# ctxnn/GenConViT

Measured on AMD Instinct MI355X. Metric: frames/sec (224x224, ed+vae forward), higher is better.
Workload: dtype f16

## Files before the change

genconvit_amd/_lib.py:

```python
from __future__ import annotations

import ctypes
import ctypes.util
import json
import os
import threading

_HERE = os.path.dirname(os.path.abspath(__file__))
LIB_PATH = os.environ.get("GCV_LIB_PATH") or os.path.join(_HERE, "lib", "libgenconvit_hip.so")

GCV_F32, GCV_BF16, GCV_F16 = 0, 1, 2
ACT_NONE, ACT_RELU, ACT_GELU, ACT_LEAKY = 0, 1, 2, 3
A_PLAIN, A_IM2COL3_POOL, A_IM2COL3_S2 = 0, 1, 2
EPI_BIAS_ACT, EPI_RESID, EPI_POOL4, EPI_CONVT, EPI_SPLITK = 0, 1, 2, 3, 4

c_void_p, c_int, c_int64, c_float, c_char_p, c_size_t = (ctypes.c_void_p, ctypes.c_int, ctypes.c_int64,
                                                         ctypes.c_float, ctypes.c_char_p, ctypes.c_size_t)


class TensorDesc(ctypes.Structure):
    _fields_ = [("name", c_char_p), ("data", c_void_p), ("numel", c_int64), ("on_device", c_int)]


class GemmArgs(ctypes.Structure):
# ... 46 lines not shown
    "gcv_frame_hist": (c_int, [c_void_p, c_int, c_int, c_int, c_int, c_void_p, c_void_p]),
    "gcv_hist_diff": (c_int, [c_void_p, c_int, c_int, c_void_p, c_void_p]),
    "gcv_frame_cells": (c_int, [c_void_p, c_int, c_int, c_int, c_int, c_void_p, c_void_p]),
    "gcv_blend_fit": (c_int, [c_void_p, c_int, c_int, c_int, c_void_p, c_void_p]),
    "gcv_hist_diff_lag": (c_int, [c_void_p, c_int, c_int, c_int, c_void_p, c_void_p]),
    "gcv_face_quality": (c_int, [c_void_p, c_int, c_int, c_int, c_void_p, c_int, c_int, c_void_p, c_void_p]),
    "gcv_face_signature": (c_int, [c_void_p, c_int, c_int, c_int, c_void_p, c_int, c_void_p, c_void_p]),
    "gcv_sig_link": (c_int, [c_void_p, c_void_p, c_int, c_int, c_void_p, c_void_p]),
    "gcv_vote_segments": (c_int, [c_void_p, c_int, c_int, c_void_p, c_int, c_void_p, c_void_p]),
    "gcv_vote_windows": (c_int, [c_void_p, c_int, c_int, c_void_p, c_int, c_void_p, c_void_p, c_void_p]),
    "gcv_tap_set": (c_int, [c_void_p, c_char_p, c_void_p, c_size_t]),
    "gcv_tap_clear": (c_int, [c_void_p]),
    "gcv_tap_written": (c_int, [c_void_p, c_char_p]),
    "gcv_profile_enable": (c_int, [c_void_p, c_int]),
    "gcv_profile_report": (c_char_p, [c_void_p]),
    "gcv_k_gemm": (c_int, [c_int, c_int, c_int, ctypes.POINTER(GemmArgs), c_void_p]),
    "gcv_gemm_plan": (c_int, [c_int, c_int, c_int, ctypes.POINTER(GemmArgs), c_void_p]),
    "gcv_k_stem_ln": (c_int, [c_int, c_void_p, c_int64, c_int64, c_int64, c_int64, c_void_p, c_void_p, c_void_p,
                              c_void_p, c_void_p, c_int, c_int, c_int, c_float, c_void_p]),
    "gcv_k_stem_ln_c": (c_int, [c_int, c_void_p, c_int64, c_int64, c_int64, c_int64, c_void_p, c_void_p, c_void_p,
                                c_void_p, c_void_p, c_int, c_int, c_int, c_int, c_float, c_void_p]),
    "gcv_k_dwconv7_ln": (c_int, [c_int, c_void_p, c_void_p, c_void_p, c_void_p, c_void_p, c_void_p, c_int, c_int,
                                 c_int, c_int, c_float, c_void_p]),
    "gcv_dw_plan": (c_int, [c_int, c_int, c_int, c_int, c_int, c_int, c_void_p]),
    "gcv_convnext_res_ok": (c_int, [c_int, c_int]),
    "gcv_k_ln_patchify": (c_int, [c_int, c_void_p, c_void_p, c_void_p, c_void_p, c_int, c_int, c_int, c_int, c_float,
                                  c_void_p]),
    "gcv_k_layernorm_rows": (c_int, [c_int, c_void_p, c_void_p, c_void_p, c_void_p, c_int64, c_int, c_float, c_void_p]),
    "gcv_k_pool_ln": (c_int, [c_int, c_void_p, c_void_p, c_void_p, c_void_p, c_int, c_int, c_int, c_float, c_void_p]),
    "gcv_k_pool_ln_rows": (c_int, [c_int, c_void_p, c_void_p, c_void_p, c_void_p, c_int, c_int, c_int, c_float, c_int, c_int,
                                   c_int, c_void_p]),
    "gcv_k_conv3_first": (c_int, [c_int, c_void_p, c_int64, c_int64, c_int64, c_int64, c_void_p, c_void_p, c_void_p,
                                  c_int, c_int, c_int, c_int, c_int, c_void_p]),
    "gcv_k_convt2_small": (c_int, [c_int, c_void_p, c_void_p, c_void_p, c_void_p, c_int, c_int, c_int, c_int, c_void_p]),
    "gcv_k_reparam": (c_int, [c_int, c_void_p, c_int, c_void_p, c_void_p, c_void_p, c_void_p, c_int, c_int, c_void_p]),
    "gcv_k_head_tail": (c_int, [c_int, c_void_p, c_void_p, c_void_p, c_void_p, c_int, c_int, c_void_p]),
    "gcv_k_head_tail_splitk": (c_int, [c_int, c_void_p, c_int, c_void_p, c_int, c_void_p, c_void_p, c_void_p, c_int, c_int,
                                       c_void_p]),
    "gcv_k_resize_mse": (c_int, [c_int, c_void_p, c_void_p, c_void_p, c_void_p, c_void_p, c_int, c_void_p]),
    "gcv_k_swin_window_attn": (c_int, [c_int, c_void_p, c_void_p, c_void_p, c_int, c_int, c_int, c_int, c_int, c_int,
                                       c_void_p]),
    "gcv_k_patch_merge_ln": (c_int, [c_int, c_void_p, c_void_p, c_void_p, c_void_p, c_int, c_int, c_int, c_int, c_float,
                                     c_void_p]),
    "gcv_k_mean_tokens": (c_int, [c_int, c_void_p, c_void_p, c_int, c_int, c_int, c_void_p]),
    "gcv_k_head_bwd": (c_int, [c_int, c_void_p, c_int, c_void_p, c_void_p, c_void_p, c_void_p, c_void_p, c_void_p, c_void_p,
                               c_int, c_int, c_void_p]),
# ... 879 lines not shown
```

genconvit_amd/csrc/api.hip:

```cpp
#include "../../include/genconvit_hip.h"

#include <dlfcn.h>

#include <cstdio>
#include <cstdlib>
#include <cstring>
#include <map>
#include <mutex>
#include <set>
#include <sstream>
#include <vector>

#include "cam.h"
#include "cam_bwd.h"
#include "cnx_mlp.h"
#include "gemm.h"
#include "kernels.h"
#include "net.h"

namespace gcv {
static thread_local std::string g_err;
void set_error(const std::string& msg) { g_err = msg; }
const char* get_error() { return g_err.c_str(); }

// ... 592 lines not shown
  };
  DISPATCH_DT(dtype, put(gemm_plan<T>(p, g, a_mode, epi)));
}

int gcv_k_stem_ln(int dtype, const void* x, int64_t sb, int64_t sc, int64_t sy, int64_t sx, const float* wp,
                  const float* bias, const float* lnw, const float* lnb, void* out, int nimg, int Ho, int Wo,
                  float eps, gcv_stream s) {
  DISPATCH_DT(dtype, launch_stem_ln<T>((const T*)x, sb, sc, sy, sx, wp, bias, lnw, lnb, (T*)out, nimg, Ho, Wo, eps,
                                       (hipStream_t)s));
}

int gcv_k_stem_ln_c(int dtype, const void* x, int64_t sb, int64_t sc, int64_t sy, int64_t sx, const float* wp,
                    const float* bias, const float* lnw, const float* lnb, void* out, int nimg, int Ho, int Wo, int C,
                    float eps, gcv_stream s) {
  DISPATCH_DT(dtype, launch_stem_ln<T>((const T*)x, sb, sc, sy, sx, wp, bias, lnw, lnb, (T*)out, nimg, Ho, Wo, eps,
                                       (hipStream_t)s, C));
}

int gcv_k_dwconv7_ln(int dtype, const void* x, const float* wdw, const float* bdw, const float* lnw,
                     const float* lnb, void* y, int nimg, int H, int W, int C, float eps, gcv_stream s) {
  DISPATCH_DT(dtype, launch_dwconv7_ln<T>((const T*)x, wdw, bdw, lnw, lnb, (T*)y, nimg, H, W, C, eps, (hipStream_t)s));
}

int gcv_dw_plan(int dtype, int nimg, int H, int W, int C, int aligned, int* out5) {
  GCV_REQUIRE(out5, "null out5");
  DwPlan p;
  auto put = [&](int rc) {
    if (rc == 0) { out5[0] = (int)p.kind; out5[1] = p.grid; out5[2] = p.block; out5[3] = p.lds; out5[4] = p.band_rows; }
    return rc;
  };
  DISPATCH_DT(dtype, put(dw_plan<T>(p, nimg, H, W, C, aligned != 0)));
}

int gcv_convnext_res_ok(int arch, int res) { return cnx_res_ok(arch, res) ? 1 : 0; }

int gcv_k_ln_patchify(int dtype, const void* x, const float* w, const float* b, void* out, int nimg, int H, int W,
                      int C, float eps, gcv_stream s) {
  DISPATCH_DT(dtype, launch_ln_patchify<T>((const T*)x, w, b, (T*)out, nimg, H, W, C, eps, (hipStream_t)s));
}

int gcv_k_layernorm_rows(int dtype, const void* x, const float* w, const float* b, void* out, int64_t rows, int C,
                         float eps, gcv_stream s) {
  DISPATCH_DT(dtype, launch_layernorm_rows<T>((const T*)x, w, b, (T*)out, rows, C, eps, (hipStream_t)s));
}

int gcv_k_pool_ln(int dtype, const void* x, const float* w, const float* b, void* out, int nimg, int HW, int C,
// ... 240 lines not shown
```

genconvit_amd/csrc/dwconv_impl.h:

```cpp
#pragma once
#include <algorithm>
#include <type_traits>

#include "dwconv_mfma.h"
#include "dwconv_pair.h"
#include "dwconv_roll.h"
#include "kernels.h"

namespace gcv {

constexpr int64_t kDwMfmaMinImageRows = 14 * 256;

template <DwKind K, int C_ = 0, int N_ = 0> struct DwShape {
  static constexpr DwKind kind = K;
  static constexpr int C = C_, N = N_;
};

template <typename T, class F> int dw_select(int nimg, int H, int W, int C, bool aligned, F&& f) {
  GCV_REQUIRE(nimg > 0 && H > 0 && W > 0, "dwconv: empty");
  const int ns = W % 7 == 0 ? W / 7 : 0;
  auto go = [&](auto sh) -> int {
    typedef decltype(sh) S;
    DwPlan p;
    p.kind = S::kind; p.C = C;
    if constexpr (S::kind == DwKind::Tile) {
      const int tiles = C == 96 ? 2 : 1;
      p.block = tiles * C;
      p.lds = tiles * 49 * (C + 2) * 4;
      p.grid = cdiv(nimg * cdiv(H, 7) * cdiv(W, 7), tiles);
    } else if constexpr (S::kind == DwKind::Tiny || S::kind == DwKind::TinyPair) {
// ... 53 lines not shown
  return -3;
}

template <typename T> int dw_plan(DwPlan& p, int nimg, int H, int W, int C, bool aligned) {
  return dw_select<T>(nimg, H, W, C, aligned, [&](const DwPlan& q, auto) { p = q; return 0; });
}

template <typename T>
int launch_dwconv7_ln(const T* x, const float* wdw, const float* bdw, const float* lnw, const float* lnb, T* y,
                      int nimg, int H, int W, int C, float eps, hipStream_t s) {
  const bool aligned = ((reinterpret_cast<uintptr_t>(x) | reinterpret_cast<uintptr_t>(y)) & 15u) == 0;
  return dw_select<T>(nimg, H, W, C, aligned, [&](const DwPlan& p, auto sh) -> int {
    typedef decltype(sh) S;
    auto band = [&](auto k) {
      return dw_launch(p, k, s, x, wdw, bdw, lnw, lnb, y, H, p.band_rows, cdiv(H, p.band_rows), eps);
    };
    if constexpr (S::kind == DwKind::Roll) return band(dwconv7_ln_roll_kernel<T, S::C, S::N>);
    else if constexpr (S::kind == DwKind::Mfma) return band(dwconv7_ln_mfma_kernel<T, S::C, S::N>);
    else if constexpr (S::kind == DwKind::Pair) return band(dwconv7_ln_pair_kernel<T, S::C, S::N>);
    else return launch_dw_tile<T>(p, x, wdw, bdw, lnw, lnb, y, nimg, H, W, eps, s);
  });
}

#define GCV_INSTANTIATE_DW(T)                                                                                        \
  template int dw_plan<T>(DwPlan&, int, int, int, int, bool);                                                        \
  template int launch_dwconv7_ln<T>(const T*, const float*, const float*, const float*, const float*, T*, int, int,   \
                                    int, int, float, hipStream_t);

}
```

genconvit_amd/csrc/dwconv_mfma.h:

```cpp
#pragma once
#include "dwconv_roll.h"

namespace gcv {


template <typename T, int C, int NS> struct DwMfmaLds {
  static constexpr int W = 7 * NS;
  static constexpr int NXG = (W + 15) / 16;
  static constexpr int RP = 16 * NXG + 8;
  static constexpr int PITCH = 2 * C + 8;
  static constexpr int SLOT = RP * PITCH;
  static constexpr int IN_BYTES = 3 * SLOT;
  static constexpr int SP = C + 4;
  static constexpr int SVAL_BYTES = 2 * W * SP * 4;
  static constexpr int bytes = IN_BYTES + SVAL_BYTES;
  static constexpr int NTASK = (C / 16) * NXG;
  static constexpr int NMW = 12;
  static constexpr int TPW = NTASK / NMW;
  static constexpr int NCONV = NMW * 64;
  static constexpr int NLN = 256;
  static constexpr int NT = NCONV + NLN;
  static_assert(NTASK % NMW == 0 && TPW >= 1 && NXG % TPW == 0, "a wave's tasks are x groups of one channel group");
  static_assert(PITCH % 8 == 0 && PITCH % 32 == 8, "pitch");
};

typedef float dwm_f32x4 __attribute__((ext_vector_type(4)));
template <typename T> struct Mfma4;
template <> struct Mfma4<half_t> {
  typedef _Float16 v4 __attribute__((ext_vector_type(4)));
  static __device__ __forceinline__ dwm_f32x4 run(uint2 a, uint2 b, dwm_f32x4 c) {
    return __builtin_amdgcn_mfma_f32_4x4x4f16(__builtin_bit_cast(v4, a), __builtin_bit_cast(v4, b), c, 0, 0, 0);
  }
};
template <> struct Mfma4<bf16_t> {
  typedef short v4 __attribute__((ext_vector_type(4)));
  static __device__ __forceinline__ dwm_f32x4 run(uint2 a, uint2 b, dwm_f32x4 c) {
    return __builtin_amdgcn_mfma_f32_4x4x4bf16_1k(__builtin_bit_cast(v4, a), __builtin_bit_cast(v4, b), c, 0, 0, 0);
  }
};

template <typename T, int C, int NS>
__global__ void __launch_bounds__((DwMfmaLds<T, C, NS>::NT), 4)
dwconv7_ln_mfma_kernel(const T* __restrict__ x, const float* __restrict__ wdw ,
                       const float* __restrict__ bdw, const float* __restrict__ lnw, const float* __restrict__ lnb,
                       T* __restrict__ y, int H, int band_rows, int nbands, float eps) {
  static_assert(sizeof(T) == 2, "16-bit storage (fp32 storage: dwconv_roll.h)");
  typedef DwElem<T> EL;
  typedef DwMfmaLds<T, C, NS> LY;
  constexpr int NCONV = LY::NCONV, NLN = LY::NLN;
  constexpr int W = LY::W, P = W, NXG = LY::NXG, TPW = LY::TPW, PITCH = LY::PITCH, SLOT = LY::SLOT, SP = LY::SP;
  constexpr int EPC = EL::EPC;
  extern __shared__ __attribute__((aligned(16))) unsigned char dwm_lds[];
  unsigned char* const in_ring = dwm_lds;
  float* const sval_ring = reinterpret_cast<float*>(dwm_lds + LY::IN_BYTES);

  const int tid = threadIdx.x;
  const int wg = xcd_remap(blockIdx.x, gridDim.x);
  const int band = wg % nbands, img = wg / nbands;
  const int ob = band * band_rows;
  const int nrows = min(band_rows, H - ob);
  const int r0 = ob - 3;
  const int nit = nrows + 6;
  const int it0 = max(0, -r0);
  constexpr int row_bytes = W * C * (int)sizeof(T);
  const int64_t img_elems = (int64_t)H * W * C;
  auto row_ok = [&](int it) { const int r = r0 + it; return it < nit && r >= 0 && r < H; };

  for (int i = tid; i < LY::IN_BYTES / 16; i += LY::NT) reinterpret_cast<u32x4*>(in_ring)[i] = u32x4{0u, 0u, 0u, 0u};
  __syncthreads();

  if (tid < NCONV) {
    const int lane = tid & 63;
    const int wave = __builtin_amdgcn_readfirstlane(tid >> 6);
    const int t0 = wave * TPW;
    const int cg = t0 / NXG, xg0 = t0 % NXG;
    const int cb = lane >> 2, n = lane & 3;
    const int c = 16 * cg + cb;
    uint2 ta[7][3];
#pragma unroll
    for (int ky = 0; ky < 7; ++ky)
// ... 195 lines not shown
      __builtin_amdgcn_sched_barrier(0);
    };

    if (row_ok(it0)) { stage_load(it0); stage_write(0); }
    if (row_ok(it0 + 1)) { stage_load(it0 + 1); stage_write(1); }
    if (row_ok(it0 + 2)) stage_load(it0 + 2);
    GCV_LDS_BARRIER();
    int wslot = 2;
    for (int it = it0; it < nit; ++it) {
      if (row_ok(it + 2)) stage_write(wslot);
      wslot = (wslot == 2) ? 0 : wslot + 1;
      if (row_ok(it + 3)) stage_load(it + 3);
      DW_STAMP(lid == 0 && it == GCV_DW_STAMP_IT, 8); DW_STAMP(lid == 0 && it == GCV_DW_STAMP_IT, 9); DW_STAMP(lid == 0 && it == GCV_DW_STAMP_IT, 10);
      DW_STAMP(lid == NLN - 64 && it == GCV_DW_STAMP_IT, 26);
      if (it >= 7) ln_row(ob + it - 7, (it - 1) & 1);
      DW_STAMP(lid == 0 && it == GCV_DW_STAMP_IT, 13); DW_STAMP(lid == NLN - 64 && it == GCV_DW_STAMP_IT, 27);
      GCV_LDS_BARRIER();
      DW_STAMP(lid == 0 && it == GCV_DW_STAMP_IT, 14); DW_STAMP(lid == NLN - 64 && it == GCV_DW_STAMP_IT, 28);
    }
    ln_row(ob + nit - 7, (nit - 1) & 1);
  }
}

}
```

genconvit_amd/csrc/dwconv_roll.h:

```cpp
#pragma once
#include <type_traits>

#include "common.h"

namespace gcv {

template <typename T> struct DwElem;
template <> struct DwElem<float> {
  static constexpr int EPC = 4;
  __device__ static __forceinline__ u32x4 pack(const float (&v)[4]) {
    return u32x4{__builtin_bit_cast(uint32_t, v[0]), __builtin_bit_cast(uint32_t, v[1]),
                 __builtin_bit_cast(uint32_t, v[2]), __builtin_bit_cast(uint32_t, v[3])};
  }
};
template <> struct DwElem<half_t> {
  static constexpr int EPC = 8;
  __device__ static __forceinline__ float lo(uint32_t v) { return (float)__builtin_bit_cast(_Float16, (uint16_t)v); }
  __device__ static __forceinline__ float hi(uint32_t v) { return (float)__builtin_bit_cast(_Float16, (uint16_t)(v >> 16)); }
};
template <> struct DwElem<bf16_t> {
  static constexpr int EPC = 8;
  __device__ static __forceinline__ float lo(uint32_t v) { return __builtin_bit_cast(float, v << 16); }
  __device__ static __forceinline__ float hi(uint32_t v) { return __builtin_bit_cast(float, v & 0xffff0000u); }
};
// ... 24 lines not shown
  asm volatile("ds_read_b32 %0, %1 offset:%2" : "=v"(dst) : "v"(addr), "n"(OFF));
}
template <int C, int S, int S1> __device__ __forceinline__ void dw_read_row(float (&nxt)[13], uint32_t addr) {
  if constexpr (S < S1) {
    static_assert(S * C * 4 < 65536, "ds offset field");
    dw_lds_rd<S * C * 4>(nxt[S], addr);
    dw_read_row<C, S + 1, S1>(nxt, addr);
  }
}

template <typename T, int C, int NS> struct DwRollLds {
  static constexpr int P = 7 * NS;
  static constexpr int HP = (NS == 1) ? 0 : 3;
  static constexpr int IN_ROW = (P + 2 * HP) * C;
  static constexpr int IN_BYTES = 3 * IN_ROW * 4;
  static constexpr int SVAL_BYTES = 2 * P * C * 4;
  static constexpr int bytes = IN_BYTES + SVAL_BYTES;
  static constexpr int NCONV = NS * C;
  static constexpr int NLN = NCONV / 3;
  static constexpr int NT = NCONV + NLN;
};

template <typename T, int C, int NS>
__global__ void __launch_bounds__((DwRollLds<T, C, NS>::NT), 4)
dwconv7_ln_roll_kernel(const T* __restrict__ x, const float* __restrict__ wdw ,
                       const float* __restrict__ bdw, const float* __restrict__ lnw, const float* __restrict__ lnb,
                       T* __restrict__ y, int H, int band_rows, int nbands, float eps) {
  typedef DwElem<T> EL;
  typedef DwRollLds<T, C, NS> LY;
  constexpr bool FULLW = (NS == 1);
  constexpr int NCONV = LY::NCONV, NLN = LY::NLN;
  constexpr int W = 7 * NS;
  constexpr int P = LY::P, HP = LY::HP, IN_ROW = LY::IN_ROW;
  constexpr int EPC = EL::EPC;
  constexpr int S0 = FULLW ? 3 : 0, S1 = FULLW ? 10 : 13;
  extern __shared__ __attribute__((aligned(16))) unsigned char dwr_lds[];
  float* const in_ring = reinterpret_cast<float*>(dwr_lds);
  float* const sval_ring = reinterpret_cast<float*>(dwr_lds + LY::IN_BYTES);

  const int tid = threadIdx.x;
  const int wg = xcd_remap(blockIdx.x, gridDim.x);
  const int band = wg % nbands, img = wg / nbands;
  const int ob = band * band_rows;
  const int nrows = min(band_rows, H - ob);
  const int r0 = ob - 3;
  const int nit = nrows + 6;
  const int it0 = max(0, -r0);
  constexpr int row_bytes = W * C * (int)sizeof(T);
  const int64_t img_elems = (int64_t)H * W * C;

  auto row_ok = [&](int it) { const int r = r0 + it; return it < nit && r >= 0 && r < H; };

  if (tid < NCONV) {
    const int sl = tid / C, c = tid - sl * C;
    auto tap_waves = [&](auto s0c, auto s1c) {
    constexpr int ES0 = decltype(s0c)::value, ES1 = decltype(s1c)::value;
    float w[49];
#pragma unroll
    for (int k = 0; k < 49; ++k) w[k] = wdw[k * C + c];
    const float bv = bdw[c];
    float acc[7][7];
#pragma unroll
    for (int i = 0; i < 7; ++i)
#pragma unroll
// ... 205 lines not shown
    };

    if (row_ok(it0)) { stage_load(it0); stage_write(0); }
    if (row_ok(it0 + 1)) { stage_load(it0 + 1); stage_write(1); }
    if (!(GCV_DWR_ABLATE & 8) && row_ok(it0 + 2)) stage_load(it0 + 2);
    GCV_LDS_BARRIER();
    int wslot = 2;
    for (int it = it0; it < nit; ++it) {
      DW_STAMP(lid == 0 && it == GCV_DW_STAMP_IT, 8); DW_STAMP(lid == NLN - 64 && it == GCV_DW_STAMP_IT, 26);
      if (!(GCV_DWR_ABLATE & 8) && row_ok(it + 2)) stage_write(wslot);
      wslot = (wslot == 2) ? 0 : wslot + 1;
      DW_STAMP(lid == 0 && it == GCV_DW_STAMP_IT, 9);
      if (!(GCV_DWR_ABLATE & 8) && row_ok(it + 3)) stage_load(it + 3);
      DW_STAMP(lid == 0 && it == GCV_DW_STAMP_IT, 10);
      if (!(GCV_DWR_ABLATE & 2) && it >= 7) ln_row(ob + it - 7, (it - 1) & 1);
      DW_STAMP(lid == 0 && it == GCV_DW_STAMP_IT, 13); DW_STAMP(lid == NLN - 64 && it == GCV_DW_STAMP_IT, 27);
      if (!(GCV_DWR_ABLATE & 16)) GCV_LDS_BARRIER();
      DW_STAMP(lid == 0 && it == GCV_DW_STAMP_IT, 14); DW_STAMP(lid == NLN - 64 && it == GCV_DW_STAMP_IT, 28);
    }
    if (!(GCV_DWR_ABLATE & 2)) ln_row(ob + nit - 7, (nit - 1) & 1);
  }
}

}
```

genconvit_amd/csrc/kernels.h:

```cpp
#pragma once
#include "common.h"

namespace gcv {

template <typename T> int launch_stem_ln(const T* x, int64_t sb, int64_t sc, int64_t sy, int64_t sx, const float* wp,
                                         const float* bias, const float* lnw, const float* lnb, T* out, int nimg,
                                         int Ho, int Wo, float eps, hipStream_t s, int C = 96);
enum class DwKind { Tile, Tiny, TinyPair, Roll, Mfma, Pair };
struct DwPlan {
  DwKind kind = DwKind::Tile;
  int C = 0, n = 0;
  int band_rows = 0;
  int grid = 0, block = 0, lds = 0;
};
template <typename T> int dw_plan(DwPlan& p, int nimg, int H, int W, int C, bool aligned);
template <typename T> int launch_dwconv7_ln(const T* x, const float* wdw, const float* bdw, const float* lnw,
                                            const float* lnb, T* y, int nimg, int H, int W, int C, float eps,
                                            hipStream_t s);
template <typename T> int launch_dw_tile(const DwPlan& p, const T* x, const float* wdw, const float* bdw, const float* lnw,
                                         const float* lnb, T* y, int nimg, int H, int W, float eps, hipStream_t s);
template <class K, class... A> int dw_launch(const DwPlan& p, K kernel, hipStream_t s, A... args) {
  if (p.lds > 64 * 1024) GCV_ENSURE_LDS(kernel, p.lds);
  hipLaunchKernelGGL(kernel, dim3(p.grid), dim3(p.block), p.lds, s, args...);
  GCV_CHECK_HIP(hipGetLastError());
  return 0;
}
template <typename T> int launch_ln_patchify(const T* x, const float* w, const float* b, T* out, int nimg, int H,
                                             int W, int C, float eps, hipStream_t s);
template <typename T> int launch_layernorm_rows(const T* x, const float* w, const float* b, T* out, int64_t rows,
                                                int C, float eps, hipStream_t s);
template <typename T> int launch_pool_ln(const T* x, const float* w, const float* b, T* out, int nimg, int HW, int C,
                                         float eps, hipStream_t s, int seg_n = 0, int row_stride = 1, int row0 = 0);
template <typename T> int launch_conv3_first(const T* x, int64_t sb, int64_t sc, int64_t sy, int64_t sx,
                                             const float* wp, const float* bias, T* out, int nimg, int H, int W,
                                             bool pool, int act, hipStream_t s);
template <typename T> int launch_convt2_small(const T* x, const float* wp, const float* bias, T* out, int nimg, int H,
                                              int W, int act, hipStream_t s);
template <typename T> int launch_reparam(const float* partial, int splitk, const float* bias, const float* eps,
                                         float* mu_out, T* z_nhwc, int B, int N, hipStream_t s);
template <typename T> int launch_head_tail(const T* h, const float* w, const float* bias, float* logits, int B, int K,
                                           hipStream_t s);
// ... 42 lines not shown
```

genconvit_amd/csrc/kernels_dev.h:

```cpp
#pragma once
#include "common.h"
#include "gemm.h"

namespace gcv {

template <typename T> __device__ __forceinline__ uint32_t bits16(float v) {
  const T t = from_f<T>(v);
  return (uint32_t)__builtin_bit_cast(unsigned short, t);
}
template <typename T> __device__ __forceinline__ float from_bits16(uint32_t u) {
  return to_f(__builtin_bit_cast(T, (unsigned short)u));
}

template <int C> constexpr int stem_tok() { return 256 / (C / 12) * 4; }
constexpr int kStemTok = stem_tok<96>();
template <typename T, int C = 96>
__global__ void __launch_bounds__(256) stem_ln_kernel(const T* __restrict__ x, int64_t sb, int64_t sc, int64_t sy,
                                                      int64_t sx, const float* __restrict__ wp,
                                                      const float* __restrict__ bias, const float* __restrict__ lnw,
                                                      const float* __restrict__ lnb, T* __restrict__ out, int nimg,
                                                      int Ho, int Wo, float eps) {
  static_assert(C == 96 || C == 192, "stem widths of ConvNeXt-T / -L");
  constexpr int TOK = stem_tok<C>(), CG = C / 12;
  __shared__ __attribute__((aligned(16))) float sW[48 * C];
// ... 309 lines not shown
    q = group32_sum(q);
    if (gl == 0) {
      stats[2 * p] = mean;
      stats[2 * p + 1] = 1.0f / sqrtf(q * (1.0f / C) + eps);
    }
  }
  __syncthreads();

  if (tile_ok) {
    const float lw = lnw[c], lb = lnb[c];
    T* yb = y + (int64_t)b * H * W * C + c;
#pragma unroll
    for (int p = 0; p < 49; ++p) {
      const int oy = y0 + p / 7, ox = x0 + p % 7;
      if (oy < H && ox < W) {
        const float mean = stats[2 * (tslot * 49 + p)], rstd = stats[2 * (tslot * 49 + p) + 1];
        yb[((int64_t)oy * W + ox) * C] = from_f<T>((acc[p] - mean) * rstd * lw + lb);
      }
    }
  }
}

template <typename T, int C, int S>
__global__ void __launch_bounds__(C) dwconv7_ln_tiny_kernel(const T* __restrict__ x, const float* __restrict__ wdw ,
                                                            const float* __restrict__ bdw, const float* __restrict__ lnw,
                                                            const float* __restrict__ lnb, T* __restrict__ y, float eps) {
  static_assert(S >= 1 && S <= 4 && C % 64 == 0, "tiny maps");
  constexpr int NPX = S * S, NW = C / 64;
  __shared__ float part[2][NW][NPX];
  const int c = threadIdx.x, wave = c >> 6, lane = c & 63;
  const T* xb = x + (int64_t)blockIdx.x * NPX * C + c;
  float xin[NPX], acc[NPX];
#pragma unroll
  for (int p = 0; p < NPX; ++p) xin[p] = to_f(xb[p * C]);
  const float bv = bdw[c];
#pragma unroll
  for (int p = 0; p < NPX; ++p) acc[p] = bv;
#pragma unroll
  for (int dy = -(S - 1); dy <= S - 1; ++dy)
#pragma unroll
    for (int dx = -(S - 1); dx <= S - 1; ++dx) {
      const float w = wdw[((dy + 3) * 7 + dx + 3) * C + c];
#pragma unroll
      for (int oy = 0; oy < S; ++oy)
#pragma unroll
        for (int ox = 0; ox < S; ++ox)
          if (oy + dy >= 0 && oy + dy < S && ox + dx >= 0 && ox + dx < S)
            acc[oy * S + ox] = fmaf(xin[(oy + dy) * S + ox + dx], w, acc[oy * S + ox]);
    }
  float mean[NPX], rstd[NPX];
#pragma unroll
  for (int p = 0; p < NPX; ++p) {
    const float sp = wave_sum(acc[p]);
    if (lane == 0) part[0][wave][p] = sp;
  }
  __syncthreads();
#pragma unroll
  for (int p = 0; p < NPX; ++p) {
    float t = 0.0f;
#pragma unroll
    for (int w = 0; w < NW; ++w) t += part[0][w][p];
    mean[p] = t * (1.0f / C);
    const float d = acc[p] - mean[p];
    const float qp = wave_sum(d * d);
    if (lane == 0) part[1][wave][p] = qp;
  }
  __syncthreads();
  const float lw = lnw[c], lb = lnb[c];
  T* yb = y + (int64_t)blockIdx.x * NPX * C + c;
#pragma unroll
  for (int p = 0; p < NPX; ++p) {
    float t = 0.0f;
#pragma unroll
    for (int w = 0; w < NW; ++w) t += part[1][w][p];
    rstd[p] = rsqrtf(t * (1.0f / C) + eps);
    yb[p * C] = from_f<T>((acc[p] - mean[p]) * rstd[p] * lw + lb);
  }
}

template <typename T>
__global__ void __launch_bounds__(256) ln_patchify_kernel(const T* __restrict__ x, const float* __restrict__ w,
                                                          const float* __restrict__ bvec, T* __restrict__ out,
                                                          int nimg, int H, int W, int C, float eps) {
  const int wave = threadIdx.x >> 6, lane = threadIdx.x & 63;
  const int64_t pix = (int64_t)blockIdx.x * 4 + wave;
  const int64_t total = (int64_t)nimg * H * W;
  if (pix >= total) return;
  const int ix = (int)(pix % W);
  const int64_t t = pix / W;
  const int iy = (int)(t % H);
  const int64_t b = t / H;
  const int Ho = H >> 1, Wo = W >> 1;
  if (iy >= 2 * Ho || ix >= 2 * Wo) return;
  const T* src = x + pix * C;
  float v[12];
  float s = 0.0f;
#pragma unroll
  for (int k = 0; k < 12; ++k) {
    const int c = lane + 64 * k;
    v[k] = (c < C) ? to_f(src[c]) : 0.0f;
// ... 891 lines not shown
```

genconvit_amd/csrc/net_impl.h:

```cpp
#pragma once
#include <algorithm>
#include <cmath>
#include <cstdlib>
#include <cstring>

#include "cam.h"
#include "cam_bwd.h"
#include "cnx_mlp.h"
#include "gemm.h"
#include "kernels.h"
#include "net.h"
#include "swin.h"

namespace gcv {

template <typename T> inline T host_cvt(float v);
template <> inline float host_cvt<float>(float v) { return v; }
template <> inline half_t host_cvt<half_t>(float v) { return (half_t)v; }
template <> inline bf16_t host_cvt<bf16_t>(float v) {
  uint32_t u;
  std::memcpy(&u, &v, 4);
  uint16_t h;
  if ((u & 0x7fffffffu) > 0x7f800000u) h = (uint16_t)((u >> 16) | 0x40);
  else h = (uint16_t)((u + 0x7fffu + ((u >> 16) & 1u)) >> 16);
// ... 628 lines not shown
          wd[s] /= 2;
          m[s] = (int64_t)segs[s].n * h[s] * wd[s];
          moff[s] = noff[s];
        }
        M = newM;
        GemmArgs g{};
        if (save3 && i == 3) Xc = X3[0];
        g.A = lnp_fused ? Hd : Y; g.lda = 4 * Cp; g.Wt = w.down[i - 1].w; g.C = Xc; g.ldc = C; g.bias = w.down[i - 1].b;
        lnp_fused = false;
        g.M = (int)M; g.N = C; g.K = 4 * Cp; g.act = ACT_NONE; g.splitk = 1;
        if (tp) GCV_TRY(tap_bb(*tp, nseg, "s" + std::to_string(i) + ".down_in", 2, i, (const T*)g.A));
        GCV_TRY(gemm("cnx.down_gemm", g, A_PLAIN, EPI_BIAS_ACT));
      }
      auto tap_block = [&](int j) {
        return tp && !lnp_fused ? tap_bb(*tp, nseg, "s" + std::to_string(i) + ".b" + std::to_string(j), 1, i, Xc) : 0;
      };
      for (int j = 0; j < A.depths[i]; ++j, ++bi) {
        const CnxBlockW<T>& k = w.blk[bi];
        T* Xn = Xc;
        if (save3 && i == 3) {
          for (int s = 0; s < nseg; ++s) segs[s].in3->x[j] = Xc + moff[s] * C;
          Xn = X3[j + 1];
        }
        for (int s = 0; s < nseg;) {
          int e = s + 1, nimg = segs[s].n;
          int64_t mm = m[s];
          while (e < nseg && h[e] == h[s] && wd[e] == wd[s]) { nimg += segs[e].n; mm += m[e]; ++e; }
          GCV_TRY(run("cnx.dwconv7_ln", 2.0 * 49 * mm * C, 2.0 * sizeof(T) * (double)mm * C + 49.0 * C * 4, [&] {
            return launch_dwconv7_ln<T>(Xc + moff[s] * C, k.dw_w, k.dw_b, k.ln_w, k.ln_b, Y + moff[s] * C, nimg, h[s],
                                        wd[s], C, 1e-6f, cur);
          }));
          s = e;
        }
        LnpSpec l;
        const bool fuse = j == A.depths[i] - 1 && i < 3 && lnp_plan(l, k.mlp.kind, C, M, nseg, segn, h, wd);
        if (fuse) { l.w = w.down[i].ln_w; l.b = w.down[i].ln_b; l.eps = 1e-6f; }
        GCV_TRY(launch_cnx_mlp<T>(*this, k.mlp, C, Y, Xc, fuse ? Hd : Xn, Hd, (int)M, fuse ? &l : nullptr, cur));
        Xc = Xn;
        lnp_fused = fuse;
        GCV_TRY(tap_block(j));
      }
    }
    bool one_fc = nseg > 1;
    for (int s = 1; s < nseg && one_fc; ++s)
      one_fc = segs[s].n == segs[0].n && segs[s].out == segs[0].out + 1000 * s && segs[s].out_ld == 1000 * nseg &&
               segs[0].out_ld == 1000 * nseg && segs[s].act == segs[0].act;
    int no = 0;
    for (int s = 0; s < nseg; ++s) {
      if (s == 0 || h[s] * wd[s] != h[s - 1] * wd[s - 1]) {
        int e = s, nimg = 0;
        int64_t mm = 0;
        while (e < nseg && h[e] * wd[e] == h[s] * wd[s]) { nimg += segs[e].n; mm += m[e]; ++e; }
        GCV_TRY(run("cnx.pool_ln", 2.0 * mm * C3, sizeof(T) * (double)mm * C3, [&] {
          if (one_fc)
            return launch_pool_ln<T>(Xc + moff[s] * C3, w.head_lnw, w.head_lnb, Pool, nimg, h[s] * wd[s], C3, 1e-6f, cur,
// ... 447 lines not shown
```

include/genconvit_hip.h:

```cpp
#ifndef GENCONVIT_HIP_H
#define GENCONVIT_HIP_H

#include <stddef.h>
#include <stdint.h>

#ifdef __cplusplus
extern "C" {
#endif

#if defined(GCV_BUILD)
#pragma GCC visibility push(default)
#endif

typedef struct gcv_handle gcv_handle;
typedef void* gcv_stream;

enum { GCV_F32 = 0, GCV_BF16 = 1, GCV_F16 = 2 };
enum { GCV_CONVNEXT_TINY = 0, GCV_CONVNEXT_LARGE = 1 };
enum { GCV_LARGE_MAX_BATCH = 256 };
enum { GCV_ACT_NONE = 0, GCV_ACT_RELU = 1, GCV_ACT_GELU = 2, GCV_ACT_LEAKY = 3 };

typedef struct {
  const char* name;
  const void* data;
// ... 100 lines not shown
int gcv_tap_set(gcv_handle* h, const char* name, void* dst, size_t bytes);
int gcv_tap_clear(gcv_handle* h);
int gcv_tap_written(gcv_handle* h, const char* name);

enum { GCV_A_PLAIN = 0, GCV_A_IM2COL3_POOL = 1, GCV_A_IM2COL3_S2 = 2 };
enum { GCV_EPI_BIAS_ACT = 0, GCV_EPI_RESID = 1, GCV_EPI_POOL4 = 2, GCV_EPI_CONVT = 3, GCV_EPI_SPLITK = 4 };

typedef struct {
  const void* A; const void* Wt; void* C;
  const float* bias; const float* gamma; const void* resid; float* partial;
  int M, N, K, lda, ldc, act, splitk, k_per_split, H, W, cin_log2, cout_log2;
} gcv_gemm_args;

int gcv_k_gemm(int dtype, int a_mode, int epi, const gcv_gemm_args* a, gcv_stream s);
int gcv_gemm_plan(int dtype, int a_mode, int epi, const gcv_gemm_args* a, int* out10);
int gcv_k_stem_ln(int dtype, const void* x, int64_t sb, int64_t sc, int64_t sy, int64_t sx, const float* wp,
                  const float* bias, const float* lnw, const float* lnb, void* out, int nimg, int Ho, int Wo,
                  float eps, gcv_stream s);
int gcv_k_stem_ln_c(int dtype, const void* x, int64_t sb, int64_t sc, int64_t sy, int64_t sx, const float* wp,
                    const float* bias, const float* lnw, const float* lnb, void* out, int nimg, int Ho, int Wo, int C,
                    float eps, gcv_stream s);
int gcv_k_dwconv7_ln(int dtype, const void* x, const float* wdw, const float* bdw, const float* lnw,
                     const float* lnb, void* y, int nimg, int H, int W, int C, float eps, gcv_stream s);
int gcv_dw_plan(int dtype, int nimg, int H, int W, int C, int aligned, int* out5);
int gcv_convnext_res_ok(int arch, int res);
int gcv_k_ln_patchify(int dtype, const void* x, const float* w, const float* b, void* out, int nimg, int H, int W,
                      int C, float eps, gcv_stream s);
int gcv_k_layernorm_rows(int dtype, const void* x, const float* w, const float* b, void* out, int64_t rows, int C,
                         float eps, gcv_stream s);
int gcv_k_pool_ln(int dtype, const void* x, const float* w, const float* b, void* out, int nimg, int HW, int C,
                  float eps, gcv_stream s);
int gcv_k_pool_ln_rows(int dtype, const void* x, const float* w, const float* b, void* out, int nimg, int HW, int C,
                       float eps, int seg_n, int row_stride, int row0, gcv_stream s);
int gcv_k_conv3_first(int dtype, const void* x, int64_t sb, int64_t sc, int64_t sy, int64_t sx, const float* wp,
                      const float* bias, void* out, int nimg, int H, int W, int pool, int act, gcv_stream s);
int gcv_k_convt2_small(int dtype, const void* x, const float* wp, const float* bias, void* out, int nimg, int H,
                       int W, int act, gcv_stream s);
int gcv_k_reparam(int dtype, const float* partial, int splitk, const float* bias, const float* eps, float* mu_out,
                  void* z_nhwc, int B, int N, gcv_stream s);
int gcv_k_head_tail(int dtype, const void* h, const float* w, const float* bias, float* logits, int B, int K,
                    gcv_stream s);
int gcv_k_head_tail_splitk(int dtype, const float* partial, int splitk, const float* b1, int act, const float* w,
                           const float* bias, float* logits, int B, int K, gcv_stream s);
int gcv_k_resize_mse(int dtype, const void* xhat, const void* img, void* recon, float* msepart, float* mse, int B,
                     gcv_stream s);

// ... 45 lines not shown
```

Before: 19010.

## Merge two-resolution depthwise conv+LN segments into one grouped kernel launch

Turns the roll, MFMA and tiny depthwise-conv+LayerNorm kernels into device-body functions, then adds a combined kernel that sends each workgroup to one of two segment groups by block index. When a ConvNeXt block handles exactly two resolution groups with compatible shapes, one launch now covers both. The aim is to remove a kernel launch and the tail underfill between two small back-to-back dwconv launches. In exchange the merged kernel takes the larger block size and LDS of the two variants, which may lower occupancy for the smaller one.

```diff
diff --git a/genconvit_amd/_lib.py b/genconvit_amd/_lib.py
--- a/genconvit_amd/_lib.py
+++ b/genconvit_amd/_lib.py
@@ -92,6 +92,8 @@
                                 c_void_p, c_void_p, c_int, c_int, c_int, c_int, c_float, c_void_p]),
     "gcv_k_dwconv7_ln": (c_int, [c_int, c_void_p, c_void_p, c_void_p, c_void_p, c_void_p, c_void_p, c_int, c_int,
                                  c_int, c_int, c_float, c_void_p]),
+    "gcv_k_dwconv7_ln2": (c_int, [c_int, c_void_p, c_void_p, c_int, c_int, c_int, c_void_p, c_void_p, c_int, c_int, c_int,
+                                  c_void_p, c_void_p, c_void_p, c_void_p, c_int, c_float, c_void_p]),
     "gcv_dw_plan": (c_int, [c_int, c_int, c_int, c_int, c_int, c_int, c_void_p]),
     "gcv_convnext_res_ok": (c_int, [c_int, c_int]),
     "gcv_k_ln_patchify": (c_int, [c_int, c_void_p, c_void_p, c_void_p, c_void_p, c_int, c_int, c_int, c_int, c_float,
diff --git a/genconvit_amd/csrc/api.hip b/genconvit_amd/csrc/api.hip
--- a/genconvit_amd/csrc/api.hip
+++ b/genconvit_amd/csrc/api.hip
@@ -638,6 +638,13 @@
   DISPATCH_DT(dtype, launch_dwconv7_ln<T>((const T*)x, wdw, bdw, lnw, lnb, (T*)y, nimg, H, W, C, eps, (hipStream_t)s));
 }
 
+int gcv_k_dwconv7_ln2(int dtype, const void* x0, void* y0, int nimg0, int H0, int W0, const void* x1, void* y1,
+                      int nimg1, int H1, int W1, const float* wdw, const float* bdw, const float* lnw, const float* lnb,
+                      int C, float eps, gcv_stream s) {
+  DISPATCH_DT(dtype, launch_dwconv7_ln2<T>((const T*)x0, (T*)y0, nimg0, H0, W0, (const T*)x1, (T*)y1, nimg1, H1, W1, wdw,
+                                           bdw, lnw, lnb, C, eps, (hipStream_t)s));
+}
+
 int gcv_dw_plan(int dtype, int nimg, int H, int W, int C, int aligned, int* out5) {
   GCV_REQUIRE(out5, "null out5");
   DwPlan p;
diff --git a/genconvit_amd/csrc/dwconv_impl.h b/genconvit_amd/csrc/dwconv_impl.h
--- a/genconvit_amd/csrc/dwconv_impl.h
+++ b/genconvit_amd/csrc/dwconv_impl.h
@@ -6,6 +6,7 @@
 #include "dwconv_pair.h"
 #include "dwconv_roll.h"
 #include "kernels.h"
+#include "kernels_dev.h"
 
 namespace gcv {
 
@@ -105,9 +106,115 @@
   });
 }
 
+template <typename T> struct DwGroupArgs {
+  const T* x;
+  T* y;
+  int H, band_rows, nbands;
+};
+
+template <typename T, class S> struct DwBody;
+template <typename T, int C, int N> struct DwBody<T, DwShape<DwKind::Roll, C, N>> {
+  static constexpr int NT = DwRollLds<T, C, N>::NT, lds = DwRollLds<T, C, N>::bytes;
+  __device__ static __forceinline__ void run(unsigned char* l, int bid, int nwg, const DwGroupArgs<T>& a, const float* wdw,
+                                             const float* bdw, const float* lnw, const float* lnb, float eps) {
+    dwconv7_ln_roll_body<T, C, N>(l, bid, nwg, a.x, wdw, bdw, lnw, lnb, a.y, a.H, a.band_rows, a.nbands, eps);
+  }
+};
+template <typename T, int C, int N> struct DwBody<T, DwShape<DwKind::Mfma, C, N>> {
+  static constexpr int NT = DwMfmaLds<T, C, N>::NT, lds = DwMfmaLds<T, C, N>::bytes;
+  __device__ static __forceinline__ void run(unsigned char* l, int bid, int nwg, const DwGroupArgs<T>& a, const float* wdw,
+                                             const float* bdw, const float* lnw, const float* lnb, float eps) {
+    dwconv7_ln_mfma_body<T, C, N>(l, bid, nwg, a.x, wdw, bdw, lnw, lnb, a.y, a.H, a.band_rows, a.nbands, eps);
+  }
+};
+template <typename T, int C, int S> struct DwBody<T, DwShape<DwKind::Tiny, C, S>> {
+  static constexpr int NT = C, lds = 0;
+  __device__ static __forceinline__ void run(unsigned char*, int bid, int, const DwGroupArgs<T>& a, const float* wdw,
+                                             const float* bdw, const float* lnw, const float* lnb, float eps) {
+    dwconv7_ln_tiny_body<T, C, S>(bid, a.x, wdw, bdw, lnw, lnb, a.y, eps);
+  }
+};
+
+template <class S0, class S1> constexpr bool dw_two_roll_pair() {
+  return S0::kind == DwKind::Roll && S1::kind == DwKind::Roll && S0::C == S1::C && S0::N == 2 * S1::N &&
+         S0::N * S0::C == 768 && S0::C != 96;
+}
+template <class S0> constexpr bool dw_two_tiny_pair() { return S0::kind == DwKind::Roll && S0::C == 768 && S0::N == 1; }
+constexpr int kDwTwoTinyS = 3;
+
+template <typename T, class S0, class S1>
+__global__ void __launch_bounds__((DwBody<T, S0>::NT > DwBody<T, S1>::NT ? DwBody<T, S0>::NT : DwBody<T, S1>::NT), 4)
+dwconv7_ln_two_kernel(const DwGroupArgs<T> a0, const DwGroupArgs<T> a1, const int grid0, const float* __restrict__ wdw,
+                      const float* __restrict__ bdw, const float* __restrict__ lnw, const float* __restrict__ lnb, float eps) {
+  typedef DwBody<T, S0> B0;
+  typedef DwBody<T, S1> B1;
+  constexpr int NT = B0::NT > B1::NT ? B0::NT : B1::NT;
+  static_assert(B0::NT % 64 == 0 && B1::NT % 64 == 0, "whole waves leave");
+  extern __shared__ __attribute__((aligned(16))) unsigned char dw2_lds[];
+  const int bx = blockIdx.x;
+  const int t0 = __builtin_amdgcn_readfirstlane((int)threadIdx.x);
+  if (bx >= grid0) {
+    if (B1::NT == NT || t0 < B1::NT) B1::run(dw2_lds, bx - grid0, (int)gridDim.x - grid0, a1, wdw, bdw, lnw, lnb, eps);
+    __builtin_amdgcn_endpgm();
+  }
+  if (B0::NT == NT || t0 < B0::NT) B0::run(dw2_lds, bx, grid0, a0, wdw, bdw, lnw, lnb, eps);
+}
+
+template <class S0, class S1, class F, class G> int dw_two_dispatch(const DwPlan& p0, const DwPlan& p1, F& f, G& g) {
+  if constexpr (dw_two_roll_pair<S0, S1>()) {
+    return f(p0, S0{}, p1, S1{});
+  } else if constexpr (dw_two_tiny_pair<S0>() && S1::kind == DwKind::Tiny) {
+    return p1.n == kDwTwoTinyS ? f(p0, S0{}, p1, DwShape<DwKind::Tiny, 768, kDwTwoTinyS>{}) : g();
+  } else {
+    return g();
+  }
+}
+
+template <typename T, class F, class G>
+int dw_select2(int nimg0, int H0, int W0, bool al0, int nimg1, int H1, int W1, bool al1, int C, F&& f, G&& g) {
+  return dw_select<T>(nimg0, H0, W0, C, al0, [&](const DwPlan& p0, auto sh0) -> int {
+    return dw_select<T>(nimg1, H1, W1, C, al1, [&](const DwPlan& p1, auto sh1) -> int {
+      return dw_two_dispatch<decltype(sh0), decltype(sh1)>(p0, p1, f, g);
+    });
+  });
+}
+
+template <typename T> bool dw_two_merged(int nimg0, int H0, int W0, int nimg1, int H1, int W1, int C, bool aligned) {
+  return dw_select2<T>(nimg0, H0, W0, aligned, nimg1, H1, W1, aligned, C,
+                       [](const DwPlan&, auto, const DwPlan&, auto) { return 1; }, [] { return 0; }) == 1;
+}
+
+template <typename T>
+int launch_dwconv7_ln2(const T* x0, T* y0, int nimg0, int H0, int W0, const T* x1, T* y1, int nimg1, int H1, int W1,
+                       const float* wdw, const float* bdw, const float* lnw, const float* lnb, int C, float eps,
+                       hipStream_t s) {
+  auto al = [](const T* x, const T* y) { return ((reinterpret_cast<uintptr_t>(x) | reinterpret_cast<uintptr_t>(y)) & 15u) == 0; };
+  return dw_select2<T>(
+      nimg0, H0, W0, al(x0, y0), nimg1, H1, W1, al(x1, y1), C,
+      [&](const DwPlan& p0, auto sh0, const DwPlan& p1, auto sh1) -> int {
+        typedef DwBody<T, decltype(sh0)> B0;
+        typedef DwBody<T, decltype(sh1)> B1;
+        DwPlan p = p0;
+        p.grid = p0.grid + p1.grid;
+        p.block = std::max(B0::NT, B1::NT);
+        p.lds = std::max(B0::lds, B1::lds);
+        const DwGroupArgs<T> a0{x0, y0, H0, p0.band_rows, p0.band_rows ? cdiv(H0, p0.band_rows) : 0};
+        const DwGroupArgs<T> a1{x1, y1, H1, p1.band_rows, p1.band_rows ? cdiv(H1, p1.band_rows) : 0};
+        return dw_launch(p, dwconv7_ln_two_kernel<T, decltype(sh0), decltype(sh1)>, s, a0, a1, p0.grid, wdw, bdw, lnw, lnb,
+                         eps);
+      },
+      [&]() -> int {
+        GCV_TRY(launch_dwconv7_ln<T>(x0, wdw, bdw, lnw, lnb, y0, nimg0, H0, W0, C, eps, s));
+        return launch_dwconv7_ln<T>(x1, wdw, bdw, lnw, lnb, y1, nimg1, H1, W1, C, eps, s);
+      });
+}
+
 #define GCV_INSTANTIATE_DW(T)                                                                                        \
   template int dw_plan<T>(DwPlan&, int, int, int, int, bool);                                                        \
   template int launch_dwconv7_ln<T>(const T*, const float*, const float*, const float*, const float*, T*, int, int,   \
-                                    int, int, float, hipStream_t);
-
-}
+                                    int, int, float, hipStream_t);                                                   \
+  template bool dw_two_merged<T>(int, int, int, int, int, int, int, bool);                                           \
+  template int launch_dwconv7_ln2<T>(const T*, T*, int, int, int, const T*, T*, int, int, int, const float*,         \
+                                     const float*, const float*, const float*, int, float, hipStream_t);
+
+}
diff --git a/genconvit_amd/csrc/dwconv_mfma.h b/genconvit_amd/csrc/dwconv_mfma.h
--- a/genconvit_amd/csrc/dwconv_mfma.h
+++ b/genconvit_amd/csrc/dwconv_mfma.h
@@ -40,22 +40,22 @@
 };
 
 template <typename T, int C, int NS>
-__global__ void __launch_bounds__((DwMfmaLds<T, C, NS>::NT), 4)
-dwconv7_ln_mfma_kernel(const T* __restrict__ x, const float* __restrict__ wdw ,
-                       const float* __restrict__ bdw, const float* __restrict__ lnw, const float* __restrict__ lnb,
-                       T* __restrict__ y, int H, int band_rows, int nbands, float eps) {
+__device__ __forceinline__ void
+dwconv7_ln_mfma_body(unsigned char* const dwm_lds, const int bid, const int nwg, const T* __restrict__ x,
+                     const float* __restrict__ wdw , const float* __restrict__ bdw,
+                     const float* __restrict__ lnw, const float* __restrict__ lnb, T* __restrict__ y, int H,
+                     int band_rows, int nbands, float eps) {
   static_assert(sizeof(T) == 2, "16-bit storage (fp32 storage: dwconv_roll.h)");
   typedef DwElem<T> EL;
   typedef DwMfmaLds<T, C, NS> LY;
   constexpr int NCONV = LY::NCONV, NLN = LY::NLN;
   constexpr int W = LY::W, P = W, NXG = LY::NXG, TPW = LY::TPW, PITCH = LY::PITCH, SLOT = LY::SLOT, SP = LY::SP;
   constexpr int EPC = EL::EPC;
-  extern __shared__ __attribute__((aligned(16))) unsigned char dwm_lds[];
   unsigned char* const in_ring = dwm_lds;
   float* const sval_ring = reinterpret_cast<float*>(dwm_lds + LY::IN_BYTES);
 
   const int tid = threadIdx.x;
-  const int wg = xcd_remap(blockIdx.x, gridDim.x);
+  const int wg = xcd_remap(bid, nwg);
   const int band = wg % nbands, img = wg / nbands;
   const int ob = band * band_rows;
   const int nrows = min(band_rows, H - ob);
@@ -297,4 +297,13 @@
   }
 }
 
+template <typename T, int C, int NS>
+__global__ void __launch_bounds__((DwMfmaLds<T, C, NS>::NT), 4)
+dwconv7_ln_mfma_kernel(const T* __restrict__ x, const float* __restrict__ wdw ,
+                       const float* __restrict__ bdw, const float* __restrict__ lnw, const float* __restrict__ lnb,
+                       T* __restrict__ y, int H, int band_rows, int nbands, float eps) {
+  extern __shared__ __attribute__((aligned(16))) unsigned char dwm_lds[];
+  dwconv7_ln_mfma_body<T, C, NS>(dwm_lds, blockIdx.x, gridDim.x, x, wdw, bdw, lnw, lnb, y, H, band_rows, nbands, eps);
 }
+
+}
diff --git a/genconvit_amd/csrc/dwconv_roll.h b/genconvit_amd/csrc/dwconv_roll.h
--- a/genconvit_amd/csrc/dwconv_roll.h
+++ b/genconvit_amd/csrc/dwconv_roll.h
@@ -70,10 +70,11 @@
 };
 
 template <typename T, int C, int NS>
-__global__ void __launch_bounds__((DwRollLds<T, C, NS>::NT), 4)
-dwconv7_ln_roll_kernel(const T* __restrict__ x, const float* __restrict__ wdw ,
-                       const float* __restrict__ bdw, const float* __restrict__ lnw, const float* __restrict__ lnb,
-                       T* __restrict__ y, int H, int band_rows, int nbands, float eps) {
+__device__ __forceinline__ void
+dwconv7_ln_roll_body(unsigned char* const dwr_lds, const int bid, const int nwg, const T* __restrict__ x,
+                     const float* __restrict__ wdw , const float* __restrict__ bdw,
+                     const float* __restrict__ lnw, const float* __restrict__ lnb, T* __restrict__ y, int H,
+                     int band_rows, int nbands, float eps) {
   typedef DwElem<T> EL;
   typedef DwRollLds<T, C, NS> LY;
   constexpr bool FULLW = (NS == 1);
@@ -82,12 +83,11 @@
   constexpr int P = LY::P, HP = LY::HP, IN_ROW = LY::IN_ROW;
   constexpr int EPC = EL::EPC;
   constexpr int S0 = FULLW ? 3 : 0, S1 = FULLW ? 10 : 13;
-  extern __shared__ __attribute__((aligned(16))) unsigned char dwr_lds[];
   float* const in_ring = reinterpret_cast<float*>(dwr_lds);
   float* const sval_ring = reinterpret_cast<float*>(dwr_lds + LY::IN_BYTES);
 
   const int tid = threadIdx.x;
-  const int wg = xcd_remap(blockIdx.x, gridDim.x);
+  const int wg = xcd_remap(bid, nwg);
   const int band = wg % nbands, img = wg / nbands;
   const int ob = band * band_rows;
   const int nrows = min(band_rows, H - ob);
@@ -339,4 +339,13 @@
   }
 }
 
-}
+template <typename T, int C, int NS>
+__global__ void __launch_bounds__((DwRollLds<T, C, NS>::NT), 4)
+dwconv7_ln_roll_kernel(const T* __restrict__ x, const float* __restrict__ wdw ,
+                       const float* __restrict__ bdw, const float* __restrict__ lnw, const float* __restrict__ lnb,
+                       T* __restrict__ y, int H, int band_rows, int nbands, float eps) {
+  extern __shared__ __attribute__((aligned(16))) unsigned char dwr_lds[];
+  dwconv7_ln_roll_body<T, C, NS>(dwr_lds, blockIdx.x, gridDim.x, x, wdw, bdw, lnw, lnb, y, H, band_rows, nbands, eps);
+}
+
+}
diff --git a/genconvit_amd/csrc/kernels.h b/genconvit_amd/csrc/kernels.h
--- a/genconvit_amd/csrc/kernels.h
+++ b/genconvit_amd/csrc/kernels.h
@@ -17,6 +17,10 @@
 template <typename T> int launch_dwconv7_ln(const T* x, const float* wdw, const float* bdw, const float* lnw,
                                             const float* lnb, T* y, int nimg, int H, int W, int C, float eps,
                                             hipStream_t s);
+template <typename T> bool dw_two_merged(int nimg0, int H0, int W0, int nimg1, int H1, int W1, int C, bool aligned);
+template <typename T> int launch_dwconv7_ln2(const T* x0, T* y0, int nimg0, int H0, int W0, const T* x1, T* y1, int nimg1,
+                                             int H1, int W1, const float* wdw, const float* bdw, const float* lnw,
+                                             const float* lnb, int C, float eps, hipStream_t s);
 template <typename T> int launch_dw_tile(const DwPlan& p, const T* x, const float* wdw, const float* bdw, const float* lnw,
                                          const float* lnb, T* y, int nimg, int H, int W, float eps, hipStream_t s);
 template <class K, class... A> int dw_launch(const DwPlan& p, K kernel, hipStream_t s, A... args) {
diff --git a/genconvit_amd/csrc/kernels_dev.h b/genconvit_amd/csrc/kernels_dev.h
--- a/genconvit_amd/csrc/kernels_dev.h
+++ b/genconvit_amd/csrc/kernels_dev.h
@@ -355,14 +355,14 @@
 }
 
 template <typename T, int C, int S>
-__global__ void __launch_bounds__(C) dwconv7_ln_tiny_kernel(const T* __restrict__ x, const float* __restrict__ wdw ,
-                                                            const float* __restrict__ bdw, const float* __restrict__ lnw,
-                                                            const float* __restrict__ lnb, T* __restrict__ y, float eps) {
+__device__ __forceinline__ void dwconv7_ln_tiny_body(const int img, const T* __restrict__ x, const float* __restrict__ wdw ,
+                                                     const float* __restrict__ bdw, const float* __restrict__ lnw,
+                                                     const float* __restrict__ lnb, T* __restrict__ y, float eps) {
   static_assert(S >= 1 && S <= 4 && C % 64 == 0, "tiny maps");
   constexpr int NPX = S * S, NW = C / 64;
   __shared__ float part[2][NW][NPX];
   const int c = threadIdx.x, wave = c >> 6, lane = c & 63;
-  const T* xb = x + (int64_t)blockIdx.x * NPX * C + c;
+  const T* xb = x + (int64_t)img * NPX * C + c;
   float xin[NPX], acc[NPX];
 #pragma unroll
   for (int p = 0; p < NPX; ++p) xin[p] = to_f(xb[p * C]);
@@ -400,7 +400,7 @@
   }
   __syncthreads();
   const float lw = lnw[c], lb = lnb[c];
-  T* yb = y + (int64_t)blockIdx.x * NPX * C + c;
+  T* yb = y + (int64_t)img * NPX * C + c;
 #pragma unroll
   for (int p = 0; p < NPX; ++p) {
     float t = 0.0f;
@@ -409,6 +409,13 @@
     rstd[p] = rsqrtf(t * (1.0f / C) + eps);
     yb[p * C] = from_f<T>((acc[p] - mean[p]) * rstd[p] * lw + lb);
   }
+}
+
+template <typename T, int C, int S>
+__global__ void __launch_bounds__(C) dwconv7_ln_tiny_kernel(const T* __restrict__ x, const float* __restrict__ wdw ,
+                                                            const float* __restrict__ bdw, const float* __restrict__ lnw,
+                                                            const float* __restrict__ lnb, T* __restrict__ y, float eps) {
+  dwconv7_ln_tiny_body<T, C, S>(blockIdx.x, x, wdw, bdw, lnw, lnb, y, eps);
 }
 
 template <typename T>
diff --git a/genconvit_amd/csrc/net_impl.h b/genconvit_amd/csrc/net_impl.h
--- a/genconvit_amd/csrc/net_impl.h
+++ b/genconvit_amd/csrc/net_impl.h
@@ -674,15 +674,33 @@
           for (int s = 0; s < nseg; ++s) segs[s].in3->x[j] = Xc + moff[s] * C;
           Xn = X3[j + 1];
         }
-        for (int s = 0; s < nseg;) {
-          int e = s + 1, nimg = segs[s].n;
-          int64_t mm = m[s];
-          while (e < nseg && h[e] == h[s] && wd[e] == wd[s]) { nimg += segs[e].n; mm += m[e]; ++e; }
-          GCV_TRY(run("cnx.dwconv7_ln", 2.0 * 49 * mm * C, 2.0 * sizeof(T) * (double)mm * C + 49.0 * C * 4, [&] {
-            return launch_dwconv7_ln<T>(Xc + moff[s] * C, k.dw_w, k.dw_b, k.ln_w, k.ln_b, Y + moff[s] * C, nimg, h[s],
-                                        wd[s], C, 1e-6f, cur);
+        int gs[4], gn[4], ng = 0;
+        int64_t gm[4];
+        for (int s = 0; s < nseg; ++ng) {
+          GCV_REQUIRE(ng < 4, "at most four segments");
+          int e = s + 1;
+          gs[ng] = s; gn[ng] = segs[s].n; gm[ng] = m[s];
+          while (e < nseg && h[e] == h[s] && wd[e] == wd[s]) { gn[ng] += segs[e].n; gm[ng] += m[e]; ++e; }
+          s = e;
+        }
+        auto dw_bytes = [&](int q) { return 2.0 * sizeof(T) * (double)gm[q] * C + 49.0 * C * 4; };
+        const T* gx[2] = {Xc + moff[gs[0]] * C, Xc + moff[gs[ng - 1]] * C};
+        T* gy[2] = {Y + moff[gs[0]] * C, Y + moff[gs[ng - 1]] * C};
+        const bool al2 = ((reinterpret_cast<uintptr_t>(gx[0]) | reinterpret_cast<uintptr_t>(gx[1]) |
+                           reinterpret_cast<uintptr_t>(gy[0]) | reinterpret_cast<uintptr_t>(gy[1])) & 15u) == 0;
+        if (ng == 2 && dw_two_merged<T>(gn[0], h[gs[0]], wd[gs[0]], gn[1], h[gs[1]], wd[gs[1]], C, al2)) {
+          GCV_TRY(run("cnx.dwconv7_ln", 2.0 * 49 * (gm[0] + gm[1]) * C, dw_bytes(0) + dw_bytes(1), [&] {
+            return launch_dwconv7_ln2<T>(gx[0], gy[0], gn[0], h[gs[0]], wd[gs[0]], gx[1], gy[1], gn[1], h[gs[1]], wd[gs[1]],
+                                         k.dw_w, k.dw_b, k.ln_w, k.ln_b, C, 1e-6f, cur);
           }));
-          s = e;
+        } else {
+          for (int q = 0; q < ng; ++q) {
+            const int s = gs[q];
+            GCV_TRY(run("cnx.dwconv7_ln", 2.0 * 49 * gm[q] * C, dw_bytes(q), [&] {
+              return launch_dwconv7_ln<T>(Xc + moff[s] * C, k.dw_w, k.dw_b, k.ln_w, k.ln_b, Y + moff[s] * C, gn[q], h[s],
+                                          wd[s], C, 1e-6f, cur);
+            }));
+          }
         }
         LnpSpec l;
         const bool fuse = j == A.depths[i] - 1 && i < 3 && lnp_plan(l, k.mlp.kind, C, M, nseg, segn, h, wd);
diff --git a/include/genconvit_hip.h b/include/genconvit_hip.h
--- a/include/genconvit_hip.h
+++ b/include/genconvit_hip.h
@@ -146,6 +146,9 @@
                     float eps, gcv_stream s);
 int gcv_k_dwconv7_ln(int dtype, const void* x, const float* wdw, const float* bdw, const float* lnw,
                      const float* lnb, void* y, int nimg, int H, int W, int C, float eps, gcv_stream s);
+int gcv_k_dwconv7_ln2(int dtype, const void* x0, void* y0, int nimg0, int H0, int W0, const void* x1, void* y1,
+                      int nimg1, int H1, int W1, const float* wdw, const float* bdw, const float* lnw, const float* lnb,
+                      int C, float eps, gcv_stream s);
 int gcv_dw_plan(int dtype, int nimg, int H, int W, int C, int aligned, int* out5);
 int gcv_convnext_res_ok(int arch, int res);
 int gcv_k_ln_patchify(int dtype, const void* x, const float* w, const float* b, void* out, int nimg, int H, int W,
diff --git a/profiles/dw_merged_bits.py b/profiles/dw_merged_bits.py
--- /dev/null
+++ b/profiles/dw_merged_bits.py
@@ -0,0 +1,43 @@
+#!/usr/bin/env python3
+import os
+import shutil
+import subprocess
+import sys
+import tempfile
+
+CONFIGS = [
+    ("genconvit b128 f16", ["--dtype", "f16"], {}),
+    ("genconvit b128 f16 serial", ["--dtype", "f16", "--no-concurrent"], {}),
+    ("genconvit b128 bf16", ["--dtype", "bf16"], {}),
+    ("genconvit b128 bf16 serial", ["--dtype", "bf16", "--no-concurrent"], {}),
+    ("vae b32 bf16", ["--net", "vae", "--batch", "32", "--dtype", "bf16"], {}),
+    ("vae b32 bf16 one stream", ["--net", "vae", "--batch", "32", "--dtype", "bf16"], {"GCV_VAE_SPLIT": "0"}),
+]
+
+
+def main():
+    import numpy as np
+    trees = {"parent": os.path.abspath(sys.argv[1]), "new": os.path.abspath(sys.argv[2])}
+    tmp = tempfile.mkdtemp(prefix="dw_merged_bits_")
+    ok = True
+    try:
+        for i, (name, args, extra) in enumerate(CONFIGS):
+            for tag, tree in trees.items():
+                lib = os.path.join(tree, "genconvit_amd", "lib", "libgenconvit_hip.so")
+                env = dict(os.environ, GCV_LIB_PATH=lib, **extra)
+                subprocess.run([sys.executable, "bench.py", "--gpus", "1", "--steps", "2", "--warmup", "1", "--no-cpu-baseline",
+                                "--dump-outputs", os.path.join(tmp, tag, str(i))] + args, check=True, env=env, cwd=tree,
+                               timeout=300, stdout=subprocess.DEVNULL, stderr=subprocess.DEVNULL)
+            for f in ("logits", "vote"):
+                a, b = (np.load(os.path.join(tmp, t, str(i), f"{f}.npy")) for t in trees)
+                same = np.array_equal(a, b) and bool(np.isfinite(a).all())
+                ok &= same
+                print(f"{name:28s} {f:7s} {str(a.shape):12s} array_equal: {same}", flush=True)
+    finally:
+        shutil.rmtree(tmp, ignore_errors=True)
+    print("ALL IDENTICAL" if ok else "MISMATCH")
+    sys.exit(0 if ok else 1)
+
+
+if __name__ == "__main__":
+    main()
```

After: 19320 (median of 6 runs). 1.6% higher.
